# RaulAstudillo06/BOCF

Hardware: AMD Instinct MI355X
Metric: acquisition evals/sec (candidates x MC-samples/sec), uEI_noiseless batch call; GP-fit ms alongside (higher is better)
Workload: dtype f64; 1 GPU; BASELINE configs[2]: m=4 rbf-ARD GP, N=4096 d=8, S=1024 MC samples, C=65536 candidates, noise 1e-06, top-16 selection; N=4096, d=8, m=4, S=1024, C=65536, rccl_ranks_seen=0

## Files before the change

bocf_amd/csrc/bocf_ctx.h:

```cpp
#pragma once
#include "bocf_internal.h"
#include "chol_plan.h"
#include "predict_plan.h"
#include "../../include/bocf_hip.h"

#include <map>
#include <string>
#include <utility>
#include <vector>

int bocf_fail(const char* what, const char* detail);
void bocf_set_error(const char* text);
int bocf_launch_status();
int bocf_plan_cholesky(bocf_ctx* c, bool kinv, CholPlan* out);
int bocf_run_cholesky(bocf_ctx* c, const CholPlan& plan, bool counters_zeroed = false);
int bocf_run_trtri(bocf_ctx* c, bool early_done);
int bocf_comm_broadcast(bocf_ctx* c, double* buf, size_t count, int root);
int bocf_comm_group(bool start);
int bocf_comm_abort(bocf_ctx* c);
int bocf_comm_allreduce_sum(bocf_ctx* c, double* buf, size_t count);
#define fail bocf_fail
#define HIPCHK(expr)                                                         \
  do {                                                                       \
    hipError_t e_ = (expr);                                                  \
// ... 27 lines not shown
    if (p) (void)hipFree(p);
    p = nullptr;
    cap = 0;
    hipError_t e = hipMalloc(&p, bytes);
    if (e != hipSuccess) return fail("hipMalloc", hipGetErrorString(e));
    cap = bytes;
    return 0;
  }
  void release() {
    if (p) (void)hipFree(p);
    p = nullptr;
    cap = 0;
  }
  template <typename T> T* as() const { return reinterpret_cast<T*>(p); }
};

struct bocf_ctx {
  int device = 0;
  hipStream_t stream = nullptr;
  void* pin_in = nullptr; void* pin_out = nullptr;
  size_t pin_in_cap = 0, pin_out_cap = 0;
  hipEvent_t ev_pin = nullptr;
  void* fit_pin = nullptr; size_t fit_pin_cap = 0;
  void* up_pin = nullptr; size_t up_pin_cap = 0, arena_used = 0;
  std::vector<hipEvent_t> ev_chol;
  hipStream_t s_res = nullptr, s_hi = nullptr, s_bulk = nullptr;
  DevBuf chol_flags;
  int chol_flags_used = 0;
  int chol_err_off = 0;
  CholOptions chol;
  int kinv_done = 0;
  int inverse_done = 0;
  int ncu = 0;
  unsigned long long* team_tl = nullptr;
  int res_cus = 0;
  int cu_masks_ok = 1;
  hipStream_t s_inv = nullptr;
  hipEvent_t ev_half = nullptr, ev_inv_early = nullptr;
  int early_inverse_started = 0;
  void* zeroed_R = nullptr; void* zeroed_RT = nullptr; int zeroed_Np = 0, zeroed_m = 0;
  int gated_off = 0;
  long long sched_timeouts = 0;
  int sched_retry = 0;
  long long fits_done = 0;
  int last_schedule = 0;
  int sched_m = 0;
  int force_sched_timeout = 0;
  int data_N = 0, data_d = 0, data_m = 0;
  int fused_infer = 1;
  int reuse_data = 0;
  int skip_mu_train = 0;
  DevBuf gpart, gout;
  DevBuf hmc_buf;
  double* infer_out = nullptr;
  size_t infer_out_cap = 0;
  bool fitted = false;
  bool canned = false;
  int N = 0, Np = 0, d = 0, m = 0, kernel_id = 0;
  long xs_stride = 0;
  std::vector<int> kernel_ids;
  std::vector<int> pending_ids;
  std::vector<KernHyp> hyp;
  std::vector<double> jitter;
  std::vector<int> last_info;
  DevBuf R32;
  bool r32_valid = false;
// ... 94 lines not shown
```

bocf_amd/csrc/bocf_internal.h:

```cpp
#pragma once
#include <hip/hip_runtime.h>
#include <stdint.h>

#define BOCF_TILE 128
#define BOCF_MAX_D 32
#define BOCF_MAX_M 16
#define BOCF_MAX_FITS 1024
#define BOCF_MAX_L 32

void bocf_note_launch(const char* kernel, hipError_t e);
#define BOCF_LAUNCH(kern, grid, block, shm, stream, ...)              \
  do {                                                                \
    hipLaunchKernelGGL(kern, grid, block, shm, stream, __VA_ARGS__);  \
    bocf_note_launch(#kern, hipGetLastError());                       \
  } while (0)

__device__ __forceinline__ void dd_fma_acc(double& s, double& c, double a, double b) {
#pragma clang fp contract(off)
  const double p = a * b;
  const double e = __builtin_fma(a, b, -p);
  const double t = s + p;
  const double z = t - s;
  c += ((s - (t - z)) + (p - z)) + e;
  s = t;
// ... 29 lines not shown
  if (!kids) {
    f(0, m, kernel_id);
    return;
  }
  for (int j0 = 0; j0 < m;) {
    int j1 = j0 + 1;
    while (j1 < m && kids[j1] == kids[j0]) ++j1;
    f(j0, j1 - j0, kids[j0]);
    j0 = j1;
  }
}

struct GemmArgs {
  const double* A;  long lda;  long strideA;
  const double* B;  long ldb;  long strideB;
  const double* Cin; double* Cout; long ldc; long strideC;
  int M, Ncols, K;
  int kb, krt, kct;
  int kbeg_rt, kbeg_ct;
  int batch1;
  long strideA2, strideB2, strideC2;
  int upper_only;
  int rt_desc;
  int ct_desc;
  int swizzle;
  int batch;
  int prefetch1;
  int stagger;
  int no_x3;
  int vprobe;
  double alpha, beta;
  double* sumsq;
  long strideSumsq;
};
void launch_gemm_f64(const GemmArgs& g, int batch, int epilogue, hipStream_t s);

struct GemmArgs32 {
  const float* A; long lda; long strideA;
  const float* B; long ldb; long strideB;
  int M, Ncols, K;
  double* sumsq; long strideSumsq;
  int tile128;
};
void launch_gemm_f32_sumsq(const GemmArgs32& g, int batch, hipStream_t s);
void launch_f64_to_f32(const double* src, float* dst, long n, hipStream_t s);

struct KernHyp {
  double variance;
  double noise;
  double ymean;
  double ls[BOCF_MAX_D];
  double jitter;
};

void launch_scale_inputs(const double* X, int n, int d, const KernHyp* hyp, int m, double* Xs, long strideXs, hipStream_t s);
void launch_build_train_kernel(const double* Xs, long strideXs, int N, int Np, int d, int kernel_id, const KernHyp* hyp,
                               const double* jitter, int add_diag, double* S, long strideS, int m, hipStream_t s, const int* kids = nullptr);
void launch_tile128(const double* A, long lda, long strideA, const double* B, long ldb, long strideB, double* C, long ldc, long strideC,
                    double alpha, double beta, int m, hipStream_t s, int ntiles = 1, int K = 128, int* done = nullptr);
#ifdef BOCF_PROBES
void dbg_tl_start();
void dbg_tl_dump(const char* path);
#endif
void set_potrf_scalar(int on);
void launch_potrf_diag(double* S, long strideS, int N, int Np, int p, double* E, double* ET, long strideE, int* info, int m, hipStream_t s,
                       int* done = nullptr);
// ... 155 lines not shown
```

bocf_amd/csrc/capi.hip:

```cpp
#include "bocf_ctx.h"

#include <chrono>
#include <cmath>
#include <cstdio>
#include <cstdlib>
#include <cstring>
#include <string>
#include <vector>

static thread_local std::string g_err;
int bocf_fail(const char* what, const char* detail) {
  g_err = std::string(what) + ": " + (detail ? detail : "");
  return -1;
}
void bocf_set_error(const char* text) { g_err = text ? text : ""; }

static thread_local std::string g_launch_err;
void bocf_note_launch(const char* kernel, hipError_t e) {
  if (e != hipSuccess && g_launch_err.empty()) g_launch_err = std::string("launch of ") + kernel + ": " + hipGetErrorString(e);
}
int bocf_launch_status() {
  const hipError_t e = hipGetLastError();
  if (!g_launch_err.empty()) {
    g_err = g_launch_err;
    g_launch_err.clear();
    return -1;
  }
  if (e != hipSuccess) return fail("hipGetLastError", hipGetErrorString(e));
  return 0;
}

extern "C" int bocf_version(void) { return 100; }
extern "C" const char* bocf_last_error(void) { return g_err.c_str(); }

extern "C" int bocf_create(int device, bocf_ctx** out) {
  if (!out) return fail("bocf_create", "null out");
  int n = 0;
  HIPCHK(hipGetDeviceCount(&n));
  if (device < 0 || device >= n) return fail("bocf_create", "no such HIP device");
  HIPCHK(hipSetDevice(device));
  bocf_ctx* c = new bocf_ctx();
  c->device = device;
  hipError_t e = hipStreamCreate(&c->stream);
  if (e != hipSuccess) {
    delete c;
    return fail("hipStreamCreate", hipGetErrorString(e));
  }
  hipDeviceProp_t prop;
  e = hipGetDeviceProperties(&prop, device);
  if (e != hipSuccess) {
    delete c;
    return fail("hipGetDeviceProperties", hipGetErrorString(e));
  }
  c->ncu = prop.multiProcessorCount;
  *out = c;
  return 0;
}

static void drop_events(bocf_ctx* c) {
  for (auto& pr : c->events) {
    (void)hipEventDestroy(pr.first);
    (void)hipEventDestroy(pr.second);
  }
  c->events.clear();
}

static void drop_phases(bocf_ctx* c) {
  for (auto& kv : c->phases)
    for (auto& pr : kv.second) {
      (void)hipEventDestroy(pr.first);
      (void)hipEventDestroy(pr.second);
    }
  c->phases.clear();
}

extern "C" void bocf_destroy(bocf_ctx* c) {
  if (!c) return;
  (void)hipSetDevice(c->device);
  (void)hipStreamSynchronize(c->stream);
  (void)bocf_comm_destroy(c);
  if (c->shard_helper) bocf_destroy(c->shard_helper);
  c->shard_helper = nullptr;
  if (c->ts_helper) bocf_destroy(c->ts_helper);
  c->ts_helper = nullptr;
  for (DevBuf& b : c->ts_F) b.release();
  drop_events(c);
  drop_phases(c);
  if (c->pin_in) (void)hipHostFree(c->pin_in);
  if (c->pin_out) (void)hipHostFree(c->pin_out);
  if (c->fit_pin) (void)hipHostFree(c->fit_pin);
  if (c->up_pin) (void)hipHostFree(c->up_pin);
  if (c->ev_pin) (void)hipEventDestroy(c->ev_pin);
  if (c->eu_pin) (void)hipHostFree(c->eu_pin);
  if (c->ev_eu_pin) (void)hipEventDestroy(c->ev_eu_pin);
  DevBuf* bufs[] = {&c->R32, &c->Ri8, &c->Ri8e, &c->Ki8, &c->Ki8e, &c->X, &c->Xs, &c->S, &c->R, &c->RT, &c->E, &c->ET, &c->T, &c->yc, &c->tvec, &c->alpha, &c->lml, &c->jit, &c->hypd,
                    &c->info, &c->mu_train, &c->rvec, &c->dvec, &c->hmc_buf, &c->Xc, &c->Kstar, &c->meanpart, &c->sumsq, &c->mean, &c->var, &c->acq, &c->Vbuf, &c->dmean, &c->dvar, &c->dacq, &c->Vs, &c->Ws, &c->theta,
                    &c->prob, &c->best, &c->params, &c->Wt, &c->blk_idx, &c->blk_val, &c->out_idx, &c->out_val, &c->gpart, &c->gout, &c->pack, &c->gidx,
                    &c->gval, &c->shard_meta, &c->chol_flags, &c->eu_theta, &c->eu_rows, &c->eu_Z, &c->eu_val, &c->eu_grad,
                    &c->ts_X, &c->ts_K, &c->ts_V, &c->ts_mp, &c->ts_mu, &c->ts_Z, &c->ts_jit, &c->ts_u, &c->ts_theta, &c->ts_params, &c->ts_out};
  for (DevBuf* b : bufs) b->release();
  if (c->infer_out) (void)hipHostFree(c->infer_out);
  for (hipEvent_t ev : c->ev_chol) (void)hipEventDestroy(ev);
  for (hipStream_t st : {c->s_res, c->s_hi, c->s_bulk, c->s_inv})
    if (st) (void)hipStreamDestroy(st);
  if (c->ev_half) (void)hipEventDestroy(c->ev_half);
  if (c->ev_inv_early) (void)hipEventDestroy(c->ev_inv_early);
  (void)hipStreamDestroy(c->stream);
  delete c;
}

struct OptDesc {
  const char* name;
  long long lo, hi;
  int kind;
  void (*set)(bocf_ctx*, long long);
  bool (*extra)(long long);
  const char* what;
};
static bool opt_lookahead_ok(long long v) { return v == -1 || v == 0 || v == 2; }
#ifdef BOCF_PROBES
static bool opt_swizzle_ok(long long v) { return v == -1 || v == 0 || v == 1 || (v >= 100 && v < 164) || (v >= 256 && v <= 258); }
static bool opt_potrf_ok(long long v) { return v == 0 || (v >= 11 && v <= 14); }
#else
static bool opt_swizzle_ok(long long v) { return v == -1 || v == 0 || v == 258; }
#endif
static const OptDesc g_options[] = {
    {"chunk", 128, 1 << 24, 0, [](bocf_ctx* c, long long v) { c->chunk = (long)round_up((int)v, 128); }, nullptr, "candidates per pass (rounded up to 128)"},
    {"workspace_mb", 1, 1 << 20, 0, [](bocf_ctx* c, long long v) { c->workspace_mb = (long)v; }, nullptr, "cap of the per-pass K* workspace"},
    {"profile", 0, 1, 0, [](bocf_ctx* c, long long v) { c->profile = v != 0; }, nullptr, "HIP events around the dominant kernel and the named phases"},
    {"predict_f32", 0, 1, 1, [](bocf_ctx* c, long long v) { c->predict_f32 = v != 0; }, nullptr, "fp32 variance contraction (BASELINE configs[4])"},
    {"i8_group", 0, 64, 0, [](bocf_ctx* c, long long v) { c->i8_group = (int)v; }, nullptr, "predict_i8: 0 = workgroups in blocks of 4 row-tile pairs x 8 column tiles per XCD; g >= 1 = bands of g pairs x all column tiles"},
    {"predict_i8", 0, 1, 1, [](bocf_ctx* c, long long v) { c->predict_i8 = v != 0; }, nullptr, "variance contraction in exact int8 products (six radix-254 digits per operand column, fp64 recombination)"},
    {"fused_infer", 0, 1, 0, [](bocf_ctx* c, long long v) { c->fused_infer = v != 0; }, nullptr, "one fused launch per inference for N <= 128"},
    {"reuse_data", 0, 1, 1, [](bocf_ctx* c, long long v) { c->reuse_data = v != 0; }, nullptr, "next fits reuse the resident X / Y"},
// ... 189 lines not shown
  launch_gemv_small_n_mfma(c->RT.as<double>(), strideS, Np, c->Vs.as<double>(), c->Ws.as<double>(), nc, c->m, c->stream);
  launch_grad_kernel(c->Xs.as<double>(), c->xs_stride, c->N, Np, c->d, c->kernel_id, c->hypd.as<KernHyp>(), c->Xc.as<double>(), s.c0, s.Cn, s.w,
                     c->Ws.as<double>(), nc, (long)Np * nc, c->dmean.as<double>(), c->dvar.as<double>(), s.p.ld, c->m, c->stream, BOCF_KIDS(c));
}

static void predict_gradients(bocf_ctx* c, const PredictPass& s) {
  const int Np = c->Np;
  GemmArgs v{};
  v.A = c->R.as<double>(); v.lda = Np; v.strideA = (long)Np * Np;
  v.B = c->Kstar.as<double>(); v.ldb = s.Cpad; v.strideB = (long)Np * s.Cpad;
  v.Cin = nullptr; v.Cout = c->Vbuf.as<double>(); v.ldc = s.Cpad; v.strideC = (long)Np * s.Cpad;
  v.M = Np; v.Ncols = s.Cpad; v.K = Np; v.kb = BOCF_TILE; v.krt = BOCF_TILE; v.rt_desc = 1; v.alpha = 1.0;
  launch_gemm_f64(v, c->m, 0, c->stream);
  GemmArgs w{};
  w.A = c->RT.as<double>(); w.lda = Np; w.strideA = (long)Np * Np;
  w.B = c->Vbuf.as<double>(); w.ldb = s.Cpad; w.strideB = (long)Np * s.Cpad;
  w.Cin = nullptr; w.Cout = c->Kstar.as<double>(); w.ldc = s.Cpad; w.strideC = (long)Np * s.Cpad;
  w.M = Np; w.Ncols = s.Cpad; w.K = Np; w.kb = Np; w.kbeg_rt = BOCF_TILE; w.alpha = 1.0;
  launch_gemm_f64(w, c->m, 0, c->stream);
  launch_grad_kernel(c->Xs.as<double>(), c->xs_stride, c->N, Np, c->d, c->kernel_id, c->hypd.as<KernHyp>(), c->Xc.as<double>(), s.c0, s.Cn, s.w,
                     c->Kstar.as<double>(), s.Cpad, (long)Np * s.Cpad, c->dmean.as<double>(), c->dvar.as<double>(), s.p.ld, c->m, c->stream, BOCF_KIDS(c));
}

static void contract_f64(bocf_ctx* c, const PredictPass& s) {
  const int Np = c->Np;
  GemmArgs g{};
  g.A = c->R.as<double>(); g.lda = Np; g.strideA = (long)Np * Np;
  g.B = c->Kstar.as<double>(); g.ldb = s.Cpad; g.strideB = (long)Np * s.Cpad;
  g.M = Np; g.Ncols = s.Cpad; g.K = Np; g.kb = BOCF_TILE; g.krt = BOCF_TILE; g.rt_desc = 1;
  g.swizzle = s.p.tiling(s.Cpad);
  g.vprobe = c->kstar_valu_probe;
  g.prefetch1 = c->prefetch1;
  g.sumsq = c->sumsq.as<double>(); g.strideSumsq = (long)s.p.nrt * s.Cpad;
  {
    KernelTimer t(c, s.Cn);
    launch_gemm_f64(g, c->m, 1, c->stream);
  }
  predict_finalize(c, s, s.p.nrt);
  if (s.need_grad) predict_gradients(c, s);
}

static void contract_f32(bocf_ctx* c, const PredictPass& s) {
  const int Np = c->Np;
  GemmArgs32 g{};
  g.A = c->R32.as<float>(); g.lda = Np; g.strideA = (long)Np * Np;
  g.B = c->Kstar.as<float>(); g.ldb = s.Cpad; g.strideB = (long)Np * s.Cpad;
  g.M = Np; g.Ncols = s.Cpad; g.K = Np;
  g.sumsq = c->sumsq.as<double>(); g.strideSumsq = (long)s.p.nrt * s.Cpad;
  g.tile128 = s.p.swizzle == 0;
  {
    KernelTimer t(c, s.Cn);
    launch_gemm_f32_sumsq(g, c->m, c->stream);
  }
  predict_finalize(c, s, s.p.nrt);
}

static void contract_i8(bocf_ctx* c, const PredictPass& s) {
  const int Np = c->Np;
  {
    KernelTimer t(c, s.Cn);
    launch_slice_operand(c->Kstar.as<double>(), s.Cpad, (long)Np * s.Cpad, Np, Np, s.Cpad, c->Ki8e.as<int>(), 0, c->Ki8.p, c->m, c->stream);
    launch_var_i8(c->Ri8.p, c->Ki8.p, Np, s.Cpad, c->Ri8e.as<int>(), c->Ki8e.as<int>(), c->sumsq.as<double>(), (long)s.p.nrt * s.Cpad, c->m, c->stream,
                  c->i8_group);
  }
  predict_finalize(c, s, s.p.nrt);
}
// ... 477 lines not shown
```

bocf_amd/csrc/gemm_f64.hip:

```cpp
#include "bocf_internal.h"

typedef double v4d __attribute__((ext_vector_type(4)));
typedef double v2d __attribute__((ext_vector_type(2)));

#define BM 128
#define BM2 256
#define BN 128
#define BK 16
#define LDT 144
#define QCH 16

template <int EPI, int PF, int NW = 4>
__global__ __launch_bounds__(64 * NW, 2) void gemm_tn_f64_kernel(GemmArgs g) {
  constexpr int JB = NW == 4 ? 4 : 2;
  constexpr int SP = 16 / NW;
  __shared__ double lds[2][2][BK][LDT];

  const int nct = g.Ncols / BN;
  const int nrt = g.M / BM;
  int b = blockIdx.x;
  int rt, ct, batch;
#ifdef BOCF_PROBES
  if (g.swizzle >= 100) {
    const int RT = g.swizzle - 100;
// ... 327 lines not shown
    if (VPROBE != 2) __syncthreads();
  }
  if (VPROBE && pacc == 1.2345e300) g.sumsq[0] = pacc;
  __syncthreads();
  double* red = &ldsA[0][0][0];
#pragma unroll
  for (int j = 0; j < 4; ++j) {
    double sq = 0.0;
#pragma unroll
    for (int i = 0; i < 4; ++i)
#pragma unroll
      for (int r = 0; r < 4; ++r) sq = __builtin_fma(acc[i][j][r], acc[i][j][r], sq);
    sq += __shfl_xor(sq, 16, 64);
    sq += __shfl_xor(sq, 32, 64);
    if (lq == 0) red[wr * 128 + wc * 64 + j * 16 + l15] = sq;
  }
  __syncthreads();
  if (tid < 256) {
    const int half = tid >> 7, col = tid & 127;
    double* out = g.sumsq + (long)batch * g.strideSumsq + (long)(rtA + half) * g.Ncols + (long)ct * BN;
    out[col] = red[(2 * half) * 128 + col] + red[(2 * half + 1) * 128 + col];
  }
}

#endif

template <int V>
struct IC {
  static constexpr int value = V;
};

#define LDA3 256
#define LDT3 128
template <int STORE>
__global__ __launch_bounds__(512, 1) void gemm_tn_f64_sumsq256x3_kernel(GemmArgs g) {
  __shared__ __attribute__((aligned(16))) double ldsA[3 * BK * LDA3];
  __shared__ __attribute__((aligned(16))) double ldsB[3 * BK * LDT3];
  const int nct = g.Ncols / BN;
  const int nrt2 = g.M / BM2;
  const int b = blockIdx.x;
  int rt2, ct, batch;
  if (STORE) {
    const int per = nct * g.batch;
    rt2 = b / per;
    const int rem = b - rt2 * per;
    batch = rem / nct;
    ct = rem - batch * nct;
  } else {
    rt2 = b / nct;
    ct = b - rt2 * nct;
    batch = blockIdx.z;
  }
  if (g.rt_desc) rt2 = nrt2 - 1 - rt2;
  const int rtA = 2 * rt2;
  const int kend = BM2 * (rt2 + 1);
  const int k0 = kend - BM2;
  long offA = (long)batch * g.strideA, offB = (long)batch * g.strideB, offC = (long)batch * g.strideC;
  if (g.batch1 > 0) {
    const int z1 = batch % g.batch1, z2 = batch / g.batch1;
    offA = (long)z1 * g.strideA + (long)z2 * g.strideA2;
    offB = (long)z1 * g.strideB + (long)z2 * g.strideB2;
    offC = (long)z1 * g.strideC + (long)z2 * g.strideC2;
  }
  const double* A = g.A + offA + (long)rt2 * BM2;
  const double* B = g.B + offB + (long)ct * BN;
  const int tid = threadIdx.x;
  const int lane = tid & 63;
  const int wave = __builtin_amdgcn_readfirstlane(tid >> 6);
  const int wr = wave >> 1, wc = wave & 1;
  const int l15 = lane & 15, lq = lane >> 4;
  const int sl = tid & 15;
  const int arow = tid >> 7, swr = (tid >> 4) & 3, sh = (tid >> 6) & 1;
  const int brow = tid >> 6, sp = (tid >> 4) & 1, bw = (tid >> 5) & 1;
  const int stA = arow * LDA3 + sh * 128 + swr * 32 + sl * 2, stB = brow * LDT3 + bw * 64 + sp * 32 + sl * 2;
  const int fgA = lq * LDA3 + wr * 32 + l15 * 2, fgB = lq * LDT3 + wc * 64 + l15 * 2;
  int stA2h = (stA >> 1) + BK * LDA3, fgA2h = (fgA >> 1) + BK * LDA3;
  asm volatile("" : "+v"(stA2h), "+v"(fgA2h));
  const int stA2 = stA2h * 2, fgA2 = fgA2h * 2;

  v4d acc[4][4];
#pragma unroll
  for (int i = 0; i < 4; ++i)
#pragma unroll
    for (int j = 0; j < 4; ++j) acc[i][j] = (v4d){0.0, 0.0, 0.0, 0.0};
  v2d ra0[4], rb0[2], ra1[4], rb1[2];
  const unsigned aoff = (unsigned)(((long)arow * g.lda + sh * 128 + swr * 16 + sl) * 8);
  const unsigned boff = (unsigned)(((long)brow * g.ldb + bw * 64 + sp * 32 + sl) * 8);
  const int lda8 = g.lda * 8, ldb8 = g.ldb * 8;
  auto fetch = [&](v2d (&ra)[4], v2d (&rb)[2], const double* pa, const double* pb) {
    const __amdgpu_buffer_rsrc_t resA = __builtin_amdgcn_make_buffer_rsrc(const_cast<double*>(pa), 0, -1, 0x00020000);
    const __amdgpu_buffer_rsrc_t resB = __builtin_amdgcn_make_buffer_rsrc(const_cast<double*>(pb), 0, -1, 0x00020000);
#pragma unroll
    for (int i = 0; i < 4; ++i) {
      ra[i][0] = __builtin_bit_cast(double, __builtin_amdgcn_raw_buffer_load_b64(resA, aoff, 4 * i * lda8, 0));
      ra[i][1] = __builtin_bit_cast(double, __builtin_amdgcn_raw_buffer_load_b64(resA, aoff + 512u, 4 * i * lda8, 0));
    }
#pragma unroll
    for (int i = 0; i < 2; ++i) {
      rb[i][0] = __builtin_bit_cast(double, __builtin_amdgcn_raw_buffer_load_b64(resB, boff, 8 * i * ldb8, 0));
      rb[i][1] = __builtin_bit_cast(double, __builtin_amdgcn_raw_buffer_load_b64(resB, boff + 128u, 8 * i * ldb8, 0));
    }
  };
  auto frag = [&](double (&a)[4], double (&bb)[4], auto bufc, auto ksc) {
    constexpr int BUF = decltype(bufc)::value, ROW = BUF * BK + decltype(ksc)::value * 4;
    const double* pa = BUF == 2 ? &ldsA[(ROW - 2 * BK) * LDA3 + fgA2] : &ldsA[ROW * LDA3 + fgA];
    const v2d a01 = *reinterpret_cast<const v2d*>(pa), a23 = *reinterpret_cast<const v2d*>(pa + 128);
    const v2d b01 = *reinterpret_cast<const v2d*>(&ldsB[ROW * LDT3 + fgB]), b23 = *reinterpret_cast<const v2d*>(&ldsB[ROW * LDT3 + fgB + 32]);
    a[0] = a01[0], a[1] = a01[1], a[2] = a23[0], a[3] = a23[1];
    bb[0] = b01[0], bb[1] = b01[1], bb[2] = b23[0], bb[3] = b23[1];
  };
  double xa[4], xb[4], ya[4], yb[4];
  auto interleave = [&](auto nmc) {
    constexpr int NM = decltype(nmc)::value;
#pragma unroll
    for (int ks = 0; ks < 4; ++ks) {
      const int nmem = ks < 3 ? 10 : 4;
      const int per = NM >= nmem ? 1 : (nmem + NM - 1) / NM;
      int done = 0;
// ... 79 lines not shown
      bb[0] = b01[0], bb[1] = b01[1], bb[2] = b23[0], bb[3] = b23[1];
    };
    auto stld = [&](int i) {
      if (i < 4) {
        *reinterpret_cast<v2d*>(sa + 4 * i * LDA3) = ra[i];
        ra[i][0] = __builtin_bit_cast(double, __builtin_amdgcn_raw_buffer_load_b64(resA, aoff, 4 * i * lda8, 0));
        ra[i][1] = __builtin_bit_cast(double, __builtin_amdgcn_raw_buffer_load_b64(resA, aoff + 512u, 4 * i * lda8, 0));
      } else {
        *reinterpret_cast<v2d*>(sb + 8 * (i - 4) * LDT3) = rb[i - 4];
        rb[i - 4][0] = __builtin_bit_cast(double, __builtin_amdgcn_raw_buffer_load_b64(resB, boff, 8 * (i - 4) * ldb8, 0));
        rb[i - 4][1] = __builtin_bit_cast(double, __builtin_amdgcn_raw_buffer_load_b64(resB, boff + 128u, 8 * (i - 4) * ldb8, 0));
      }
    };
    auto k4 = [&](const double (&a)[4], const double (&bb)[4], int ks) {
#pragma unroll
      for (int q = 0; q < 4; ++q) {
        if (q >= qmin) {
#pragma unroll
          for (int j = 0; j < 4; ++j) acc[q][j] = __builtin_amdgcn_mfma_f64_16x16x4f64(a[q], bb[j], acc[q][j], 0, 0, 0);
        }
        if (ks < 3 && q < 2) stld(2 * ks + q);
      }
    };
    fragp(ya, yb, fa_c, fb_c, 1);
    k4(xa, xb, 0);
    fragp(xa, xb, fa_c, fb_c, 2);
    k4(ya, yb, 1);
    fragp(ya, yb, fa_c, fb_c, 3);
    k4(xa, xb, 2);
    fragp(xa, xb, fa_n, fb_n, 0);
    k4(ya, yb, 3);
    __syncthreads();
  };
  fetch(ra0, rb0, A, B);
  fetch(ra1, rb1, A + tileA, B + tileB);
#pragma unroll
  for (int i = 0; i < 4; ++i) *reinterpret_cast<v2d*>(&ldsA[4 * i * LDA3 + stA]) = ra0[i];
#pragma unroll
  for (int i = 0; i < 2; ++i) *reinterpret_cast<v2d*>(&ldsB[8 * i * LDT3 + stB]) = rb0[i];
  fetch(ra0, rb0, A + 2 * tileA, B + 2 * tileB);
#pragma unroll
  for (int i = 0; i < 4; ++i) *reinterpret_cast<v2d*>(&ldsA[(BK + 4 * i) * LDA3 + stA]) = ra1[i];
#pragma unroll
  for (int i = 0; i < 2; ++i) *reinterpret_cast<v2d*>(&ldsB[(BK + 8 * i) * LDT3 + stB]) = rb1[i];
  fetch(ra1, rb1, A + 3 * tileA, B + 3 * tileB);
  __syncthreads();
  frag(xa, xb, IC<0>(), IC<0>());
  const int nfull = k0 / BK, rounds = nfull / 6, rest = nfull - 6 * rounds;
  int kt = 0;
  for (int it = 0; it < rounds; ++it, kt += 6 * BK) {
    step(ra0, rb0, kt, IC<0>());
    step(ra1, rb1, kt + BK, IC<1>());
    step(ra0, rb0, kt + 2 * BK, IC<2>());
    step(ra1, rb1, kt + 3 * BK, IC<0>());
    step(ra0, rb0, kt + 4 * BK, IC<1>());
    step(ra1, rb1, kt + 5 * BK, IC<2>());
  }
  if (rest >= 2) {
    step(ra0, rb0, kt, IC<0>());
    step(ra1, rb1, kt + BK, IC<1>());
  }
  if (rest >= 4) {
    step(ra0, rb0, kt + 2 * BK, IC<2>());
    step(ra1, rb1, kt + 3 * BK, IC<0>());
  }
  {
    int cur = rest == 0 ? 0 : (rest == 2 ? 2 : 1);
    for (kt = k0; kt < kend; kt += 2 * BK) {
      dstep(ra0, rb0, kt, cur);
      cur = cur == 2 ? 0 : cur + 1;
      dstep(ra1, rb1, kt + BK, cur);
      cur = cur == 2 ? 0 : cur + 1;
    }
  }
  if (STORE) {
    double* stage = ldsA;
    double* Cout = g.Cout + offC + (long)rt2 * BM2 * g.ldc + (long)ct * BN;
    const double alpha = g.alpha;
    __syncthreads();
#pragma unroll
    for (int pass = 0; pass < 4; ++pass) {
#pragma unroll
      for (int j = 0; j < 4; ++j)
#pragma unroll
        for (int r = 0; r < 4; ++r) stage[(16 * wr + 4 * r + lq) * LDT3 + wc * 64 + 16 * j + l15] = acc[pass][j][r];
      __syncthreads();
#pragma unroll
      for (int e = 0; e < 8; ++e) {
        const int rr = wave + 8 * e;
        v2d v = *reinterpret_cast<const v2d*>(&stage[rr * LDT3 + lane * 2]);
        v[0] *= alpha;
        v[1] *= alpha;
        *reinterpret_cast<v2d*>(Cout + (long)(64 * pass + rr) * g.ldc + lane * 2) = v;
      }
      __syncthreads();
    }
    return;
  }
  double* xfer = ldsA;
  double* red = ldsA + 4 * 4 * 2 * 64;
#pragma unroll 1
  for (int stage = 0; stage < 4; ++stage) {
    if (wr == stage) {
#pragma unroll
      for (int q = 0; q < 4; ++q)
#pragma unroll
        for (int j = 0; j < 4; ++j) {
          double* slot = xfer + ((q * 4 + j) * 2 + wc) * 64 + lane;
          double sq = stage == 0 ? 0.0 : *slot;
#pragma unroll
          for (int r = 0; r < 4; ++r) sq = __builtin_fma(acc[q][j][r], acc[q][j][r], sq);
          if (stage < 3) {
            *slot = sq;
          } else {
            sq += __shfl_xor(sq, 16, 64);
            sq += __shfl_xor(sq, 32, 64);
            if (lq == 0) red[q * 128 + wc * 64 + j * 16 + l15] = sq;
          }
        }
    }
    __syncthreads();
  }
  if (tid < 256) {
    const int half = tid >> 7, col = tid & 127;
    double* out = g.sumsq + (long)batch * g.strideSumsq + (long)(rtA + half) * g.Ncols + (long)ct * BN;
    out[col] = red[(2 * half) * 128 + col] + red[(2 * half + 1) * 128 + col];
  }
}

void launch_gemm_f64(const GemmArgs& g0, int batch, int epilogue, hipStream_t s) {
  GemmArgs g = g0;
  g.batch = batch;
  const int nrt = g.M / BM, nct = g.Ncols / BN;
  if (nrt == 0 || nct == 0 || batch == 0) return;
  if (g.swizzle >= 256) {
    if (epilogue == 1 && !g.prefetch1 && g.M % BM2 == 0 && g.kbeg_rt == 0 && g.kbeg_ct == 0 && g.batch1 == 0) {
      const dim3 grid256((unsigned)((g.M / BM2) * nct), 1, (unsigned)batch);
#ifdef BOCF_PROBES
#define L256(V, A, B) BOCF_LAUNCH((gemm_tn_f64_sumsq256_kernel<V, A, B>), grid256, dim3(512), 0, s, g)
      if (g.swizzle != 258 || g.vprobe) {
        g.stagger = g.swizzle == 257 ? 1 : 0;
        if (g.vprobe == 1) L256(1, 2, 2);
        else if (g.vprobe == 2) L256(2, 2, 2);
        else if (g.vprobe == 3) L256(3, 2, 2);
        else if (g.vprobe == 4) L256(4, 2, 2);
        else if (g.stagger == 1) L256(0, 2, 0);
        else L256(0, 2, 2);
        return;
      }
#undef L256
#endif
      if (g.kb == BM && g.krt == BM && g.kct == 0 && g.K >= g.M) {
        BOCF_LAUNCH((gemm_tn_f64_sumsq256x3_kernel<0>), grid256, dim3(512), 0, s, g);
        return;
      }
    }
    g.swizzle = 0;
  }
  if (epilogue == 0 && !g.no_x3 && !g.Cin && g.M % BM2 == 0 && g.M >= 2 * BM2 && g.kb == BM && g.krt == BM && g.kct == 0 && g.kbeg_rt == 0 && g.kbeg_ct == 0 &&
      g.K >= g.M && !g.upper_only && g.rt_desc && !g.ct_desc) {
    const dim3 grid256((unsigned)((g.M / BM2) * nct * batch), 1, 1);
    BOCF_LAUNCH((gemm_tn_f64_sumsq256x3_kernel<1>), grid256, dim3(512), 0, s, g);
    return;
  }
  if (epilogue == 3) {
    BOCF_LAUNCH((gemm_tn_f64_kernel<3, 1, 8>), dim3((unsigned)(nct * (nct + 1) / 2 * batch)), dim3(512), 0, s, g);
    return;
  }
  dim3 grid((unsigned)(nrt * nct), 1, (unsigned)batch);
#ifdef BOCF_PROBES
  if (g.swizzle >= 100 && (nct % 8 != 0 || nrt % (g.swizzle - 100) != 0)) g.swizzle = 0;
  if (g.swizzle >= 100) {
    grid = dim3((unsigned)(nrt * nct * batch), 1, 1);
  } else if (g.swizzle == 1) {
    const long ns = (long)((nrt + 7) / 8) * ((nct + 7) / 8) * batch;
    grid = dim3((unsigned)(((ns + 7) / 8) * 8 * 64), 1, 1);
  }
#else
  if (g.swizzle != 2) g.swizzle = 0;
#endif
  if (g.swizzle == 2) grid = dim3((unsigned)(nrt * nct * batch), 1, 1);
  if (epilogue == 0)
    BOCF_LAUNCH((gemm_tn_f64_kernel<0, 1, 8>), grid, dim3(512), 0, s, g);
  else if (g.prefetch1)
    BOCF_LAUNCH((gemm_tn_f64_kernel<1, 1>), grid, dim3(256), 0, s, g);
  else
// ... 3 lines not shown
```

bocf_amd/csrc/predict.hip:

```cpp
#include "bocf_internal.h"
#include "../../include/bocf_hip.h"

__device__ __forceinline__ double kern_of_r2_p(int kernel_id, double variance, double r2) {
  if (kernel_id <= 1) return variance * bocf_exp_nonpos(-0.5 * r2);
  const double r = sqrt(r2);
  if (kernel_id == 2) {
    const double s5r = 2.23606797749978969641 * r;
    return variance * (1.0 + s5r + (5.0 / 3.0) * r2) * bocf_exp_nonpos(-s5r);
  }
  const double s3r = 1.73205080756887729353 * r;
  return variance * (1.0 + s3r) * bocf_exp_nonpos(-s3r);
}

typedef double v2d_p __attribute__((ext_vector_type(2)));
typedef float v2f_p __attribute__((ext_vector_type(2)));
template <int D, int KID, int STORE>
__global__ __launch_bounds__(256) void cross_kernel(const double* __restrict__ Xs, long strideXs, int N, int Np, int kernel_id_unused,
                                                    const KernHyp* __restrict__ hyp, const double* __restrict__ Xc, int c0, int Cn,
                                                    const double* __restrict__ alpha, double* __restrict__ Kstar, long ldk, long strideK,
                                                    double* __restrict__ meanpart, double* __restrict__ meanlo, int nsplit, int Cpad,
                                                    int store_k, int jbase, int mtot) {
  const int j = blockIdx.z;
  const int split = blockIdx.y;
  const int c = (blockIdx.x * 256 + threadIdx.x) * 2;
  if (c >= Cpad) return;
  const bool valid0 = c < Cn, valid1 = c + 1 < Cn;
  const KernHyp h = hyp[j];
  double xa[D], xb[D];
#pragma unroll
  for (int q = 0; q < D; ++q) {
    xa[q] = valid0 ? Xc[(long)(c0 + c) * D + q] / h.ls[q] : 0.0;
    xb[q] = valid1 ? Xc[(long)(c0 + c + 1) * D + q] / h.ls[q] : 0.0;
  }
  const int nblk = Np / BOCF_TILE;
  const int bps = (nblk + nsplit - 1) / nsplit;
  const int b0 = split * bps;
  int b1 = b0 + bps;
  if (b1 > nblk) b1 = nblk;
  const double* __restrict__ X = Xs + (long)j * strideXs;
  const double* __restrict__ al = alpha + (long)j * Np;
  double* __restrict__ Kj = Kstar + (long)j * strideK;
  float* __restrict__ Kf = reinterpret_cast<float*>(Kstar) + (long)j * strideK;
  for (int blk = b0; blk < b1; ++blk) {
    double mean0 = 0.0, mean1 = 0.0, lo0 = 0.0, lo1 = 0.0;
    const int kbeg = blk * BOCF_TILE;
    for (int kk = kbeg; kk < kbeg + BOCF_TILE; ++kk) {
      double v0 = 0.0, v1 = 0.0;
      if (kk < N) {
        double r0 = 0.0, r1 = 0.0;
#pragma unroll
        for (int q = 0; q < D; ++q) {
          const double xq = X[(long)kk * D + q];
          const double d0 = xq - xa[q], d1 = xq - xb[q];
          r0 += d0 * d0;
          r1 += d1 * d1;
        }
        v0 = kern_of_r2_p(KID, h.variance, r0);
        v1 = kern_of_r2_p(KID, h.variance, r1);
        const double a = al[kk];
        dd_fma_acc(mean0, lo0, v0, a);
        dd_fma_acc(mean1, lo1, v1, a);
      }
      if (STORE == 1) __builtin_nontemporal_store((v2d_p){valid0 ? v0 : 0.0, valid1 ? v1 : 0.0}, reinterpret_cast<v2d_p*>(Kj + (long)kk * ldk + c));
      else if (STORE == 2) __builtin_nontemporal_store((v2f_p){valid0 ? (float)v0 : 0.f, valid1 ? (float)v1 : 0.f}, reinterpret_cast<v2f_p*>(Kf + (long)kk * ldk + c));
    }
    *reinterpret_cast<v2d_p*>(meanpart + ((long)blk * mtot + jbase + j) * Cpad + c) = (v2d_p){mean0, mean1};
    *reinterpret_cast<v2d_p*>(meanlo + ((long)blk * mtot + jbase + j) * Cpad + c) = (v2d_p){lo0, lo1};
  }
}

template <int D>
static void launch_cross_d(const double* Xs, long strideXs, int N, int Np, int kernel_id, const KernHyp* hyp, const double* Xc, int c0,
                           int Cn, int Cpad, const double* alpha, double* Kstar, long ldk, long strideK, double* meanpart, double* meanlo,
                           int nsplit, int m, int store_k, hipStream_t s, int jbase, int mtot) {
  dim3 grid((unsigned)((Cpad + 511) / 512), (unsigned)nsplit, (unsigned)m);
  const int kid = kernel_id <= 1 ? 0 : kernel_id;
#define LAUNCH(KID, ST)                                                                                                        \
  BOCF_LAUNCH((cross_kernel<D, KID, ST>), grid, dim3(256), 0, s, Xs, strideXs, N, Np, kernel_id, hyp, Xc, c0, Cn, alpha, \
                     Kstar, ldk, strideK, meanpart, meanlo, nsplit, Cpad, store_k, jbase, mtot)
#define BYSTORE(KID)                          \
  if (store_k == 0) LAUNCH(KID, 0);           \
  else if (store_k == 1) LAUNCH(KID, 1);      \
  else LAUNCH(KID, 2)
  if (kid == 0) { BYSTORE(0); }
  else if (kid == 2) { BYSTORE(2); }
  else { BYSTORE(3); }
#undef BYSTORE
#undef LAUNCH
}

static void launch_cross_kernel_run(const double* Xs, long strideXs, int N, int Np, int d, int kernel_id, const KernHyp* hyp, const double* Xc, int c0, int Cn,
                                    int Cpad, const double* alpha, double* Kstar, long ldk, long strideK, double* meanpart, double* meanlo, int nsplit,
                                    int m, int store_k, hipStream_t s, int jbase, int mtot);
void launch_cross_kernel(const double* Xs, long strideXs, int N, int Np, int d, int kernel_id, const KernHyp* hyp, const double* Xc,
                         int c0, int Cn, int Cpad, const double* alpha, double* Kstar, long ldk, long strideK, double* meanpart,
                         double* meanlo, int nsplit, int m, int store_k, hipStream_t s, const int* kids) {
  int jbase = 0, mtot = m;
// ... 492 lines not shown
```

Measured before the change: 1.048 billion evals/s.

## Persistent tile-queue sumsq GEMM with cross-tile prefetch; pipeline cross-kernel row loads

```diff
diff --git a/bocf_amd/csrc/bocf_ctx.h b/bocf_amd/csrc/bocf_ctx.h
--- a/bocf_amd/csrc/bocf_ctx.h
+++ b/bocf_amd/csrc/bocf_ctx.h
@@ -83,6 +83,7 @@
   int kinv_done = 0;
   int inverse_done = 0;
   int ncu = 0;
+  int* tile_ctr = nullptr;
   unsigned long long* team_tl = nullptr;
   int res_cus = 0;
   int cu_masks_ok = 1;
diff --git a/bocf_amd/csrc/bocf_internal.h b/bocf_amd/csrc/bocf_internal.h
--- a/bocf_amd/csrc/bocf_internal.h
+++ b/bocf_amd/csrc/bocf_internal.h
@@ -85,6 +85,8 @@
   double alpha, beta;
   double* sumsq;
   long strideSumsq;
+  int* tile_ctr;
+  int ncu;
 };
 void launch_gemm_f64(const GemmArgs& g, int batch, int epilogue, hipStream_t s);
 
diff --git a/bocf_amd/csrc/capi.hip b/bocf_amd/csrc/capi.hip
--- a/bocf_amd/csrc/capi.hip
+++ b/bocf_amd/csrc/capi.hip
@@ -53,6 +53,14 @@
     return fail("hipGetDeviceProperties", hipGetErrorString(e));
   }
   c->ncu = prop.multiProcessorCount;
+  e = hipMalloc((void**)&c->tile_ctr, 2 * sizeof(int));
+  if (e == hipSuccess) e = hipMemset(c->tile_ctr, 0, 2 * sizeof(int));
+  if (e != hipSuccess) {
+    if (c->tile_ctr) (void)hipFree(c->tile_ctr);
+    (void)hipStreamDestroy(c->stream);
+    delete c;
+    return fail("bocf_create: tile counters", hipGetErrorString(e));
+  }
   *out = c;
   return 0;
 }
@@ -100,6 +108,7 @@
                     &c->ts_X, &c->ts_K, &c->ts_V, &c->ts_mp, &c->ts_mu, &c->ts_Z, &c->ts_jit, &c->ts_u, &c->ts_theta, &c->ts_params, &c->ts_out};
   for (DevBuf* b : bufs) b->release();
   if (c->infer_out) (void)hipHostFree(c->infer_out);
+  if (c->tile_ctr) (void)hipFree(c->tile_ctr);
   for (hipEvent_t ev : c->ev_chol) (void)hipEventDestroy(ev);
   for (hipStream_t st : {c->s_res, c->s_hi, c->s_bulk, c->s_inv})
     if (st) (void)hipStreamDestroy(st);
@@ -355,6 +364,7 @@
   g.vprobe = c->kstar_valu_probe;
   g.prefetch1 = c->prefetch1;
   g.sumsq = c->sumsq.as<double>(); g.strideSumsq = (long)s.p.nrt * s.Cpad;
+  g.tile_ctr = c->tile_ctr; g.ncu = c->ncu;
   {
     KernelTimer t(c, s.Cn);
     launch_gemm_f64(g, c->m, 1, c->stream);
diff --git a/bocf_amd/csrc/gemm_f64.hip b/bocf_amd/csrc/gemm_f64.hip
--- a/bocf_amd/csrc/gemm_f64.hip
+++ b/bocf_amd/csrc/gemm_f64.hip
@@ -383,15 +383,29 @@
 
 #define LDA3 256
 #define LDT3 128
-template <int STORE>
+template <int STORE, int QUEUE = 0>
 __global__ __launch_bounds__(512, 1) void gemm_tn_f64_sumsq256x3_kernel(GemmArgs g) {
+  static_assert(!(STORE && QUEUE), "the tile queue exists for the sum-of-squares epilogue only");
   __shared__ __attribute__((aligned(16))) double ldsA[3 * BK * LDA3];
   __shared__ __attribute__((aligned(16))) double ldsB[3 * BK * LDT3];
+  __shared__ int next_tile;
   const int nct = g.Ncols / BN;
   const int nrt2 = g.M / BM2;
-  const int b = blockIdx.x;
+  int b = blockIdx.x;
+  v2d ra0[4], rb0[2], ra1[4], rb1[2];
+  bool primed = false;
+  auto tile_of = [&](int t, int& rt2_, int& ct_, int& batch_) {
+    const int per = nrt2 * nct;
+    batch_ = t / per;
+    const int rem = t - batch_ * per;
+    rt2_ = rem / nct;
+    ct_ = rem - rt2_ * nct;
+  };
+ for (;;) {
   int rt2, ct, batch;
-  if (STORE) {
+  if (QUEUE) {
+    tile_of(b, rt2, ct, batch);
+  } else if (STORE) {
     const int per = nct * g.batch;
     rt2 = b / per;
     const int rem = b - rt2 * per;
@@ -434,7 +448,6 @@
   for (int i = 0; i < 4; ++i)
 #pragma unroll
     for (int j = 0; j < 4; ++j) acc[i][j] = (v4d){0.0, 0.0, 0.0, 0.0};
-  v2d ra0[4], rb0[2], ra1[4], rb1[2];
   const unsigned aoff = (unsigned)(((long)arow * g.lda + sh * 128 + swr * 16 + sl) * 8);
   const unsigned boff = (unsigned)(((long)brow * g.ldb + bw * 64 + sp * 32 + sl) * 8);
   const int lda8 = g.lda * 8, ldb8 = g.ldb * 8;
@@ -580,8 +593,10 @@
     k4(ya, yb, 3);
     __syncthreads();
   };
-  fetch(ra0, rb0, A, B);
-  fetch(ra1, rb1, A + tileA, B + tileB);
+  if (!(QUEUE && primed)) {
+    fetch(ra0, rb0, A, B);
+    fetch(ra1, rb1, A + tileA, B + tileB);
+  }
 #pragma unroll
   for (int i = 0; i < 4; ++i) *reinterpret_cast<v2d*>(&ldsA[4 * i * LDA3 + stA]) = ra0[i];
 #pragma unroll
@@ -612,6 +627,8 @@
     step(ra0, rb0, kt + 2 * BK, IC<2>());
     step(ra1, rb1, kt + 3 * BK, IC<0>());
   }
+  int claimed = 0;
+  if (QUEUE && tid == 0) claimed = (int)gridDim.x + atomicAdd(g.tile_ctr, 1);
   {
     int cur = rest == 0 ? 0 : (rest == 2 ? 2 : 1);
     for (kt = k0; kt < kend; kt += 2 * BK) {
@@ -647,6 +664,8 @@
   }
   double* xfer = ldsA;
   double* red = ldsA + 4 * 4 * 2 * 64;
+  int nb = 0;
+  if (QUEUE && tid == 0) next_tile = claimed;
 #pragma unroll 1
   for (int stage = 0; stage < 4; ++stage) {
     if (wr == stage) {
@@ -668,11 +687,33 @@
         }
     }
     __syncthreads();
+    if (QUEUE && stage == 0) {
+      nb = __builtin_amdgcn_readfirstlane(next_tile);
+      primed = nb < nrt2 * nct * g.batch;
+      if (primed) {
+        int nrt, nc, nz;
+        tile_of(nb, nrt, nc, nz);
+        if (g.rt_desc) nrt = nrt2 - 1 - nrt;
+        const double* An = g.A + (long)nz * g.strideA + (long)nrt * BM2;
+        const double* Bn = g.B + (long)nz * g.strideB + (long)nc * BN;
+        fetch(ra0, rb0, An, Bn);
+        fetch(ra1, rb1, An + tileA, Bn + tileB);
+      }
+    }
   }
   if (tid < 256) {
     const int half = tid >> 7, col = tid & 127;
     double* out = g.sumsq + (long)batch * g.strideSumsq + (long)(rtA + half) * g.Ncols + (long)ct * BN;
     out[col] = red[(2 * half) * 128 + col] + red[(2 * half + 1) * 128 + col];
+  }
+  if (!QUEUE) return;
+  if (!primed) break;
+  b = nb;
+  __syncthreads();
+ }
+  if (threadIdx.x == 0 && atomicAdd(g.tile_ctr + 1, 1) == (int)gridDim.x - 1) {
+    __hip_atomic_store(g.tile_ctr, 0, __ATOMIC_RELAXED, __HIP_MEMORY_SCOPE_AGENT);
+    __hip_atomic_store(g.tile_ctr + 1, 0, __ATOMIC_RELAXED, __HIP_MEMORY_SCOPE_AGENT);
   }
 }
 
@@ -699,7 +740,11 @@
 #undef L256
 #endif
       if (g.kb == BM && g.krt == BM && g.kct == 0 && g.K >= g.M) {
-        BOCF_LAUNCH((gemm_tn_f64_sumsq256x3_kernel<0>), grid256, dim3(512), 0, s, g);
+        const long tiles = (long)(g.M / BM2) * nct * batch;
+        if (g.tile_ctr && g.ncu > 0 && tiles <= 0x7fffffffL - g.ncu)
+          BOCF_LAUNCH((gemm_tn_f64_sumsq256x3_kernel<0, 1>), dim3((unsigned)(tiles < g.ncu ? tiles : g.ncu)), dim3(512), 0, s, g);
+        else
+          BOCF_LAUNCH((gemm_tn_f64_sumsq256x3_kernel<0>), grid256, dim3(512), 0, s, g);
         return;
       }
     }
diff --git a/bocf_amd/csrc/predict.hip b/bocf_amd/csrc/predict.hip
--- a/bocf_amd/csrc/predict.hip
+++ b/bocf_amd/csrc/predict.hip
@@ -15,7 +15,8 @@
 typedef double v2d_p __attribute__((ext_vector_type(2)));
 typedef float v2f_p __attribute__((ext_vector_type(2)));
 template <int D, int KID, int STORE>
-__global__ __launch_bounds__(256) void cross_kernel(const double* __restrict__ Xs, long strideXs, int N, int Np, int kernel_id_unused,
+__global__ __launch_bounds__(256) __attribute__((amdgpu_waves_per_eu(D <= 8 ? 8 : 1)))
+void cross_kernel(const double* __restrict__ Xs, long strideXs, int N, int Np, int kernel_id_unused,
                                                     const KernHyp* __restrict__ hyp, const double* __restrict__ Xc, int c0, int Cn,
                                                     const double* __restrict__ alpha, double* __restrict__ Kstar, long ldk, long strideK,
                                                     double* __restrict__ meanpart, double* __restrict__ meanlo, int nsplit, int Cpad,
@@ -41,28 +42,72 @@
   const double* __restrict__ al = alpha + (long)j * Np;
   double* __restrict__ Kj = Kstar + (long)j * strideK;
   float* __restrict__ Kf = reinterpret_cast<float*>(Kstar) + (long)j * strideK;
+  const bool full_cols = (int)(blockIdx.x * 512u + 511u) < Cn;
   for (int blk = b0; blk < b1; ++blk) {
     double mean0 = 0.0, mean1 = 0.0, lo0 = 0.0, lo1 = 0.0;
     const int kbeg = blk * BOCF_TILE;
-    for (int kk = kbeg; kk < kbeg + BOCF_TILE; ++kk) {
-      double v0 = 0.0, v1 = 0.0;
-      if (kk < N) {
+    if (full_cols && kbeg + BOCF_TILE <= N) {
+      auto fetch = [&](double (&xr)[D], double& a, int k) {
+#pragma unroll
+        for (int q = 0; q < D; ++q) xr[q] = X[(long)k * D + q];
+        a = al[k];
+      };
+      auto row = [&](const double (&xr)[D], double a, int kk) {
         double r0 = 0.0, r1 = 0.0;
 #pragma unroll
         for (int q = 0; q < D; ++q) {
-          const double xq = X[(long)kk * D + q];
-          const double d0 = xq - xa[q], d1 = xq - xb[q];
+          const double d0 = xr[q] - xa[q], d1 = xr[q] - xb[q];
           r0 += d0 * d0;
           r1 += d1 * d1;
         }
-        v0 = kern_of_r2_p(KID, h.variance, r0);
-        v1 = kern_of_r2_p(KID, h.variance, r1);
-        const double a = al[kk];
+        const double v0 = kern_of_r2_p(KID, h.variance, r0);
+        const double v1 = kern_of_r2_p(KID, h.variance, r1);
         dd_fma_acc(mean0, lo0, v0, a);
         dd_fma_acc(mean1, lo1, v1, a);
+        if (STORE == 1) __builtin_nontemporal_store((v2d_p){v0, v1}, reinterpret_cast<v2d_p*>(Kj + (long)kk * ldk + c));
+        else if (STORE == 2) __builtin_nontemporal_store((v2f_p){(float)v0, (float)v1}, reinterpret_cast<v2f_p*>(Kf + (long)kk * ldk + c));
+      };
+      double xA[D], aA;
+      if constexpr (D <= 8) {
+        double xB[D], aB;
+        fetch(xA, aA, kbeg);
+        for (int kk = kbeg; kk < kbeg + BOCF_TILE; kk += 2) {
+          int kn = kk + 1;
+          asm volatile("" : "+s"(kn) : "s"(xA[0]), "s"(aA));
+          fetch(xB, aB, kn);
+          row(xA, aA, kk);
+          kn = kk + 2 < kbeg + BOCF_TILE ? kk + 2 : kk + 1;
+          asm volatile("" : "+s"(kn) : "s"(xB[0]), "s"(aB));
+          fetch(xA, aA, kn);
+          row(xB, aB, kk + 1);
+        }
+      } else {
+        for (int kk = kbeg; kk < kbeg + BOCF_TILE; ++kk) {
+          fetch(xA, aA, kk);
+          row(xA, aA, kk);
+        }
       }
-      if (STORE == 1) __builtin_nontemporal_store((v2d_p){valid0 ? v0 : 0.0, valid1 ? v1 : 0.0}, reinterpret_cast<v2d_p*>(Kj + (long)kk * ldk + c));
-      else if (STORE == 2) __builtin_nontemporal_store((v2f_p){valid0 ? (float)v0 : 0.f, valid1 ? (float)v1 : 0.f}, reinterpret_cast<v2f_p*>(Kf + (long)kk * ldk + c));
+    } else {
+      for (int kk = kbeg; kk < kbeg + BOCF_TILE; ++kk) {
+        double v0 = 0.0, v1 = 0.0;
+        if (kk < N) {
+          double r0 = 0.0, r1 = 0.0;
+#pragma unroll
+          for (int q = 0; q < D; ++q) {
+            const double xq = X[(long)kk * D + q];
+            const double d0 = xq - xa[q], d1 = xq - xb[q];
+            r0 += d0 * d0;
+            r1 += d1 * d1;
+          }
+          v0 = kern_of_r2_p(KID, h.variance, r0);
+          v1 = kern_of_r2_p(KID, h.variance, r1);
+          const double a = al[kk];
+          dd_fma_acc(mean0, lo0, v0, a);
+          dd_fma_acc(mean1, lo1, v1, a);
+        }
+        if (STORE == 1) __builtin_nontemporal_store((v2d_p){valid0 ? v0 : 0.0, valid1 ? v1 : 0.0}, reinterpret_cast<v2d_p*>(Kj + (long)kk * ldk + c));
+        else if (STORE == 2) __builtin_nontemporal_store((v2f_p){valid0 ? (float)v0 : 0.f, valid1 ? (float)v1 : 0.f}, reinterpret_cast<v2f_p*>(Kf + (long)kk * ldk + c));
+      }
     }
     *reinterpret_cast<v2d_p*>(meanpart + ((long)blk * mtot + jbase + j) * Cpad + c) = (v2d_p){mean0, mean1};
     *reinterpret_cast<v2d_p*>(meanlo + ((long)blk * mtot + jbase + j) * Cpad + c) = (v2d_p){lo0, lo1};
```

Result: faster. 1.069 billion evals/s (median of 6 runs) (+2.0%).
